# saminiir/level-ip

Hardware: AMD Instinct MI355X
Metric: device-resident checksum GB/s over packet batch; % of HBM-read roofline (higher is better)
Workload: dtype u16

## Files before the change

level-ip_amd/csrc/csum_dev.h:

```cpp
#pragma once

#include <hip/hip_runtime.h>

#include <stdint.h>

#include <atomic>
#include <type_traits>

#include "flat_src.h"
#include "lvlip_csum.h"
#include "lvlip_skb.h"

namespace lvlip {


template <bool ODD>
__device__ __forceinline__ uint32_t dword_words(uint32_t x) {
    if (ODD) x = ((x & 0x00ff00ffu) << 8) | ((x >> 8) & 0x00ff00ffu);
    return (x & 0xffffu) + (x >> 16);
}

template <bool ODD>
__device__ __forceinline__ uint32_t chunk_words(const uint4 v) {
    return dword_words<ODD>(v.x) + dword_words<ODD>(v.y) + dword_words<ODD>(v.z) +
// ... 157 lines not shown
}

template <int G, int WPB = SW_WAVES>
struct Deal {
    uint64_t nw, rank, p_lo;
    uint32_t cnt;

    __device__ __forceinline__ bool init(uint32_t n, uint32_t wid) {
        nw = (uint64_t)gridDim.x * WPB;
        if (G == 0) {
            rank = (uint64_t)blockIdx.x * WPB + wid;
            const uint64_t per = ((uint64_t)n + nw - 1) / nw;
            p_lo = rank * per;
            if (p_lo >= n) return false;
            cnt = (uint32_t)min<uint64_t>(per, (uint64_t)n - p_lo);
            return true;
        }
        rank = (gridDim.x & 7u) == 0u
                   ? ((uint64_t)(blockIdx.x & 7u) * (gridDim.x >> 3) + (blockIdx.x >> 3)) * WPB + wid
                   : (uint64_t)blockIdx.x * WPB + wid;
        p_lo = 0;
        const uint64_t ng = ((uint64_t)n + G - 1) / G;
        if (rank >= ng) return false;
        const uint64_t gcount = (ng - 1 - rank) / nw + 1;
        const uint64_t glast = rank + (gcount - 1) * nw;
        const uint64_t last_size = min<uint64_t>((uint64_t)(G > 0 ? G : 1), (uint64_t)n - glast * G);
        cnt = (uint32_t)((gcount - 1) * G + last_size);
        return true;
    }
    __device__ __forceinline__ uint64_t gidx(uint32_t k) const {
        if (G == 0) return p_lo + k;
        return ((uint64_t)(k / (G > 0 ? G : 1)) * nw + rank) * G + (k % (G > 0 ? G : 1));
    }
};

template <int G, int WPB>
__device__ __forceinline__ void fetch_window(const lvlip_csum_desc* __restrict__ descs,
                                             const Deal<G, WPB>& dl, uint32_t first, uint32_t lane,
                                             uint4* win ) {
    uint32_t k = first + lane;
    k = k < dl.cnt ? k : dl.cnt - 1u;
    const lvlip_csum_desc* g = descs + dl.gidx(k);
    const uint32_t lds = (uint32_t)__builtin_amdgcn_readfirstlane(
        (int)(uint32_t)(uintptr_t)(__attribute__((address_space(3))) uint4*)win);
#pragma clang diagnostic push
#pragma clang diagnostic ignored "-Winline-asm"
    asm volatile("s_nop 4\n\ts_mov_b32 m0, %1\n\ts_nop 0\n\tglobal_load_lds_dwordx4 %0, off"
                 :
                 : "v"(g), "s"(lds)
                 : "memory", "m0");
#pragma clang diagnostic pop
}

template <int R, int G, int POL, int WPB = SW_WAVES>
__device__ __forceinline__ void ring_sweep(const uint8_t* __restrict__ base,
                                           const lvlip_csum_desc* __restrict__ descs, uint32_t n,
                                           uint16_t* __restrict__ out, uint4 (*s_win)[64]) {
    constexpr uint32_t END = 0xffffffffu;
    constexpr uint32_t PIECE = 2048u;
    const uint32_t lane = threadIdx.x & 63u;
    const uint32_t lane16 = lane * 16u;
    const uint32_t wid = uniform(threadIdx.x >> 6);
    Deal<G, WPB> dl;
    if (!dl.init(n, wid)) return;
    const uint32_t cnt = dl.cnt;

    fetch_window<G, WPB>(descs, dl, 0u, lane, s_win[0]);
    fetch_window<G, WPB>(descs, dl, 64u, lane, s_win[1]);
    asm volatile("s_waitcnt vmcnt(0)" ::: "memory");

    uint32_t m_x, m_y, m_z, m_t, m_s;
    auto load_window_meta = [&](uint32_t w) {
        const uint4 d = s_win[w & 1u][lane];
        const PacketMeta pm = packet_meta(base, u32x4{d.x, d.y, d.z, d.w});
        m_x = pm.srd.x;
        m_y = pm.srd.y;
        m_z = pm.srd.z;
        m_t = pm.tinfo;
        m_s = pm.start;
    };
    load_window_meta(0);

    uint32_t ip = 0, io = 0;
    u32x4 srd;
    uint32_t tinfo, start;
    auto pull = [&](uint32_t k) {
        srd.x = (uint32_t)__builtin_amdgcn_readlane((int)m_x, (int)k);
        srd.y = (uint32_t)__builtin_amdgcn_readlane((int)m_y, (int)k);
        srd.z = (uint32_t)__builtin_amdgcn_readlane((int)m_z, (int)k);
        srd.w = SRD_WORD3;
        tinfo = (uint32_t)__builtin_amdgcn_readlane((int)m_t, (int)k);
        start = (uint32_t)__builtin_amdgcn_readlane((int)m_s, (int)k);
    };
    pull(0);

    uint32_t gc = 0;
    uint32_t res_w = 0, res_s = 0;
    uint32_t acc = 0;
    u32x4 va[R], vb[R];
    uint32_t s_pkt[R], s_start[R], s_meta[R];

    auto issue = [&](int r) {
        const bool live = ip < cnt;
        u32x4 sr = srd;
        if (!live) sr.z = 0;
        const uint32_t off = lane16 + io;
        va[r] = buffer_load_nt_asm<POL>(off, sr);
        vb[r] = buffer_load_nt_asm<POL>(off + 1024u, sr);
        const bool last = io + PIECE >= srd.z;
        s_pkt[r] = live ? ip : END;
        s_start[r] = start;
        s_meta[r] = (uint32_t)last | ((tinfo & 3u) << 1) | (((srd.z - 4u) - io) << 3);
        if (live) {
            if (!last) {
                io += PIECE;
            } else {
                ++ip;
                io = 0;
                if (ip < cnt) {
                    if ((ip & 63u) == 0u) {
                        load_window_meta(ip >> 6);
                        fetch_window<G, WPB>(descs, dl, ip + 64u, lane, s_win[((ip >> 6) + 1u) & 1u]);
                    }
                    pull(ip & 63u);
                }
            }
        }
    };

    auto consume = [&](int r) {
        piece_wait<2 * (R - 1)>(va[r], vb[r]);
        u32x4 x = va[r], y = vb[r];
        const uint32_t meta = s_meta[r];
        const uint32_t len3 = (meta >> 1) & 3u;
        if ((meta & 1u) && len3) {
            const uint32_t pos = meta >> 3;
            const uint32_t m = (1u << (8u * len3)) - 1u;
            const bool me = lane == ((pos >> 4) & 63u);
            const uint32_t tk = (pos >> 2) & 3u;
            const bool in_b = pos >= 1024u;
            const uint32_t m0 = (me && tk == 0u) ? m : ~0u, m1 = (me && tk == 1u) ? m : ~0u;
            const uint32_t m2 = (me && tk == 2u) ? m : ~0u, m3 = (me && tk == 3u) ? m : ~0u;
            if (in_b) {
                y.x &= m0; y.y &= m1; y.z &= m2; y.w &= m3;
            } else {
                x.x &= m0; x.y &= m1; x.z &= m2; x.w &= m3;
            }
        }
        acc = dot2_acc(x.x, acc);
        acc = dot2_acc(x.y, acc);
        acc = dot2_acc(x.z, acc);
        acc = dot2_acc(x.w, acc);
        acc = dot2_acc(y.x, acc);
        acc = dot2_acc(y.y, acc);
        acc = dot2_acc(y.z, acc);
        acc = dot2_acc(y.w, acc);
        if (meta & 1u) {
            const uint32_t w = wave_sum_dpp(acc);
            acc = 0;
            const uint32_t k = s_pkt[r] - gc;
            if (lane == k) {
                res_w = w;
                res_s = s_start[r];
            }
            if (k == 63u || s_pkt[r] + 1u == cnt) {
                uint32_t tt = res_s + res_w;
                tt = (tt & 0xffffu) + (tt >> 16);
                tt = (tt & 0xffffu) + (tt >> 16);
                if (lane <= k) out[dl.gidx(gc + lane)] = (uint16_t)~tt;
                gc += 64u;
            }
        }
    };

#pragma unroll
    for (int r = 0; r < R; ++r) issue(r);
    bool done = false;
    while (!done) {
#pragma unroll
        for (int r = 0; r < R; ++r) {
            if (s_pkt[r] == END) {
                done = true;
                break;
            }
            consume(r);
            issue(r);
        }
    }
    asm volatile("s_waitcnt vmcnt(0)" ::: "memory");
}

constexpr int FT = 256;
constexpr uint32_t FCAP = 128;

template <int CTRL>
__device__ __forceinline__ uint32_t dpp_row_shr(uint32_t v) {
    return (uint32_t)__builtin_amdgcn_update_dpp(0, (int)v, CTRL, 0xF, 0xF, false);
}

__device__ __forceinline__ uint32_t wave_incl_scan(uint32_t v) {
    v += dpp_row_shr<0x111>(v);
    v += dpp_row_shr<0x112>(v);
    v += dpp_row_shr<0x114>(v);
    v += dpp_row_shr<0x118>(v);
    v += (uint32_t)__builtin_amdgcn_update_dpp(0, (int)v, 0x142, 0xA, 0xF, false);
    v += (uint32_t)__builtin_amdgcn_update_dpp(0, (int)v, 0x143, 0xC, 0xF, false);
    return v;
}

__device__ __forceinline__ u32x4 group_load_nt(uint64_t a) {
    u32x4 r;
    asm volatile("global_load_dwordx4 %0, %1, off nt" : "=v"(r) : "v"(a) : "memory");
    return r;
}

template <int N>
__device__ __forceinline__ void group_wait(u32x4& a) {
    asm volatile("s_waitcnt vmcnt(%1)" : "+v"(a) : "n"(N) : "memory");
}

__device__ __forceinline__ void block_excl_scan2(uint32_t a, uint32_t b, uint32_t* s_tmp ,
                                                 uint32_t* ea, uint32_t* eb, uint32_t* ta,
                                                 uint32_t* tb) {
    const uint32_t lane = threadIdx.x & 63u, wid = threadIdx.x >> 6;
    const uint32_t ia = wave_incl_scan(a), ib = wave_incl_scan(b);
    if (lane == 63u) {
        s_tmp[wid] = ia;
        s_tmp[4u + wid] = ib;
    }
    __syncthreads();
    uint32_t ba = 0, bb = 0, aa = 0, ab = 0;
#pragma unroll
    for (uint32_t k = 0; k < 4; ++k) {
        const uint32_t x = s_tmp[k], y = s_tmp[4u + k];
        ba += (k < wid) ? x : 0u;
        bb += (k < wid) ? y : 0u;
        aa += x;
        ab += y;
    }
    __syncthreads();
    *ea = ba + ia - a;
    *eb = bb + ib - b;
// ... 557 lines not shown
```

level-ip_amd/csrc/csum_kernels.hip:

```cpp
#include <hip/hip_runtime.h>

#include <stdint.h>
#include <stdio.h>
#include <string.h>

#include "csum_dev.h"

namespace lvlip {

template <int R, int G>
__global__ __launch_bounds__(256) void k_window(const uint8_t* __restrict__ base,
                                                const lvlip_csum_desc* __restrict__ descs,
                                                uint32_t n, uint16_t* __restrict__ out) {
    static_assert(G > 0, "k_window deals groups of G >= 1 packets");
    __shared__ uint4 s_win[SW_WAVES][2][64];
    ring_sweep<R, G, 0>(base, descs, n, out, s_win[uniform(threadIdx.x >> 6)]);
}

template <int S, int P, int K, int M>
__global__ __launch_bounds__(256) void k_lane(const uint8_t* __restrict__ base,
                                              const lvlip_csum_desc* __restrict__ descs,
                                              uint32_t n, uint16_t* __restrict__ out) {
    static_assert(S == 1 || S == 2 || S == 4 || S == 8, "lanes per packet");
    constexpr uint32_t PB = 256 / S;
    const uint32_t lane = threadIdx.x & 63u;
    const uint32_t sub = threadIdx.x & (uint32_t)(S - 1);
    const uint32_t i0 = blockIdx.x * (PB * (uint32_t)P) + threadIdx.x / (uint32_t)S;
    uint4 dd[P];
#pragma unroll
    for (int p = 0; p < P; ++p) {
        const uint32_t i = i0 + PB * p;
        if (M == 0) {
            dd[p] = i < n ? load_global(reinterpret_cast<uint64_t>(descs + i)) : make_uint4(0u, 0u, 0u, 0u);
        } else {
            const uint4 v = load_global(reinterpret_cast<uint64_t>(descs + (i < n ? i : n - 1u)));
            dd[p] = i < n ? v : make_uint4(0u, 0u, 0u, 0u);
        }
    }
    const uint64_t safe = reinterpret_cast<uint64_t>(descs);
    uint64_t a0[P];
    uint32_t lo[P], nch[P], lastv[P];
    uint4 x[P][K];
#pragma unroll
    for (int p = 0; p < P; ++p) {
        const uint64_t abs = reinterpret_cast<uint64_t>(base) + (((uint64_t)dd[p].y << 32) | dd[p].x);
        const int32_t len = (int32_t)dd[p].z;
        a0[p] = abs & ~15ull;
        lo[p] = (uint32_t)(abs & 15ull);
        const uint64_t span = (uint64_t)lo[p] + (uint64_t)(uint32_t)(len > 0 ? len : 0);
        nch[p] = len > 0 ? (uint32_t)((span + 15u) >> 4) : 0u;
        lastv[p] = len > 0 ? (uint32_t)(span - 16ull * (nch[p] - 1u)) : 16u;
        const bool in_group = nch[p] <= (uint32_t)(S * K);
#pragma unroll
        for (int k = 0; k < K; ++k) {
            const uint32_t c = sub + (uint32_t)(S * k);
            const bool want = in_group && c < nch[p];
            if (M == 0)
                x[p][k] = want ? load_nt_global(a0[p] + 16ull * c) : make_uint4(0u, 0u, 0u, 0u);
            else
                x[p][k] = load_nt_global(want ? a0[p] + 16ull * c : safe);
        }
    }
    if (M == 1) __builtin_amdgcn_sched_barrier(0);
    uint32_t acc[P];
#pragma unroll
    for (int p = 0; p < P; ++p) {
        const uint32_t sel = (lo[p] & 1u) ? 0x02030001u : 0x03020100u;
        const bool in_group = nch[p] <= (uint32_t)(S * K);
        uint32_t a = 0;
#pragma unroll
// ... 3 lines not shown
            const int b0 = c == 0u ? (int)lo[p] : 0;
            const int b1 = c + 1u == nch[p] ? (int)lastv[p] : 16;
            if (M == 1 || c == 0u || c + 1u == nch[p]) v = mask_chunk(v, b0, b1);
            a = dot2_acc(__builtin_amdgcn_perm(v.x, v.x, sel), a);
            a = dot2_acc(__builtin_amdgcn_perm(v.y, v.y, sel), a);
            a = dot2_acc(__builtin_amdgcn_perm(v.z, v.z, sel), a);
            a = dot2_acc(__builtin_amdgcn_perm(v.w, v.w, sel), a);
        }
#pragma unroll
        for (int off = 1; off < S; off <<= 1) a += __shfl_xor(a, off, 64);
        acc[p] = a;
    }
#pragma unroll
    for (int p = 0; p < P; ++p) {
        uint64_t big = __builtin_amdgcn_ballot_w64(sub == 0u && nch[p] > (uint32_t)(S * K));
        while (big) {
            const uint32_t q = (uint32_t)__builtin_ctzll(big);
            big &= big - 1ull;
            const uint64_t qa0 = ((uint64_t)(uint32_t)__builtin_amdgcn_readlane((int)(a0[p] >> 32), (int)q) << 32) |
                                 (uint32_t)__builtin_amdgcn_readlane((int)(uint32_t)a0[p], (int)q);
            const uint32_t qlo = (uint32_t)__builtin_amdgcn_readlane((int)lo[p], (int)q);
            const uint32_t qn = (uint32_t)__builtin_amdgcn_readlane((int)nch[p], (int)q);
            const uint32_t qlv = (uint32_t)__builtin_amdgcn_readlane((int)lastv[p], (int)q);
            const uint4* src = reinterpret_cast<const uint4*>(qa0);
            uint32_t w = (qlo & 1u) ? wave_packet_sum<4, true>(src, qn, (int)qlo, qlv, lane)
                                    : wave_packet_sum<4, false>(src, qn, (int)qlo, qlv, lane);
            w = wave_sum_dpp(w);
            if (lane == q) acc[p] = w;
        }
    }
#pragma unroll
    for (int p = 0; p < P; ++p) {
        const uint32_t i = i0 + PB * p;
        if (sub == 0u && i < n) out[i] = finish(dd[p].w, acc[p]);
    }
}

}


namespace {

using lvlip_host::cu_count;
using lvlip_host::current_cus;
using lvlip_host::kLaunchMax;

thread_local char g_last_err[256] = "";

int hip_fail(hipError_t e, const char* what) {
    snprintf(g_last_err, sizeof g_last_err, "%s: %s", what, hipGetErrorString(e));
    return LVLIP_EHIP;
}

template <int R, int G>
void launch_window_g(int waves_per_cu, hipStream_t s, const void* base, const lvlip_csum_desc* d,
                     uint32_t n, uint16_t* out) {
    uint64_t waves = (uint64_t)current_cus() * (uint64_t)waves_per_cu;
    const uint64_t ng = ((uint64_t)n + G - 1) / G;
    if (waves > ng) waves = ng;
    uint64_t grid = (waves + lvlip::SW_WAVES - 1) / lvlip::SW_WAVES;
    if (grid > 8) grid = grid & ~7ull;
    hipLaunchKernelGGL((lvlip::k_window<R, G>), dim3((uint32_t)grid), dim3(256), 0, s,
                       (const uint8_t*)base, d, n, out);
}

int window_group(int requested, int len_hint) {
    if (requested == 1 || requested == 2 || requested == 3 || requested == 4 || requested == 8)
        return requested;
    if (len_hint >= 4096) return 3;
    if (len_hint >= 1792) return 2;
    return 4;
}

template <int R>
void launch_window(int waves_per_cu, hipStream_t s, const void* base, const lvlip_csum_desc* d,
                   uint32_t n, uint16_t* out, int group, int len_hint) {
    switch (window_group(group, len_hint)) {
        case 1: launch_window_g<R, 1>(waves_per_cu, s, base, d, n, out); break;
        case 3: launch_window_g<R, 3>(waves_per_cu, s, base, d, n, out); break;
        case 4: launch_window_g<R, 4>(waves_per_cu, s, base, d, n, out); break;
        case 8: launch_window_g<R, 8>(waves_per_cu, s, base, d, n, out); break;
        default: launch_window_g<R, 2>(waves_per_cu, s, base, d, n, out); break;
    }
}

template <int S, int P, int K>
void launch_lane_spk(int mode, hipStream_t s, const void* base, const lvlip_csum_desc* d, uint32_t n,
                     uint16_t* out) {
    constexpr uint64_t per_block = 256 / S * P;
    const uint32_t grid = (uint32_t)(((uint64_t)n + per_block - 1) / per_block);
    if (mode)
        hipLaunchKernelGGL((lvlip::k_lane<S, P, K, 1>), dim3(grid), dim3(256), 0, s,
                           (const uint8_t*)base, d, n, out);
    else
        hipLaunchKernelGGL((lvlip::k_lane<S, P, K, 0>), dim3(grid), dim3(256), 0, s,
                           (const uint8_t*)base, d, n, out);
}

bool launch_lane(int lanes, int per_group, int chunks, int mode, hipStream_t s, const void* base,
                 const lvlip_csum_desc* d, uint32_t n, uint16_t* out) {
    switch ((lanes << 16) | (chunks << 8) | per_group) {
#define LVLIP_LANE(SS, PP, KK) \
    case (SS << 16) | (KK << 8) | PP: launch_lane_spk<SS, PP, KK>(mode, s, base, d, n, out); return true;
        LVLIP_LANE(1, 2, 4) LVLIP_LANE(1, 4, 4) LVLIP_LANE(1, 2, 6)
        LVLIP_LANE(2, 2, 2) LVLIP_LANE(2, 4, 2) LVLIP_LANE(2, 4, 1) LVLIP_LANE(2, 8, 1)
        LVLIP_LANE(2, 2, 4)
        LVLIP_LANE(4, 2, 1) LVLIP_LANE(4, 4, 1) LVLIP_LANE(4, 8, 1) LVLIP_LANE(4, 2, 2)
        LVLIP_LANE(4, 4, 2)
        LVLIP_LANE(8, 4, 1) LVLIP_LANE(8, 2, 2) LVLIP_LANE(8, 4, 2)
#undef LVLIP_LANE
        default: return false;
    }
}

constexpr int kLaneHintMax = 33;

int auto_select(int hint, uint32_t n, int* unroll, int* wpc) {
    if (hint >= 896) {
        if (*wpc <= 0) *wpc = hint < 1280 ? 16 : (hint < 1792 ? 12 : 8);
        if (*unroll <= 0) {
            const uint64_t nw = (uint64_t)current_cus() * (uint64_t)*wpc;
            int g = hint < 1792 ? 4 : (hint < 4096 ? 2 : 3);
            while (g > 1 && (uint64_t)n < 16ull * (uint64_t)g * nw) --g;
            *unroll = 2 | (g << 8);
        }
        return LVLIP_KERNEL_WINDOW;
    }
    if (hint > 0 && hint < kLaneHintMax) {
        *unroll = 4 | (2 << 8) | (2 << 16);
        return LVLIP_KERNEL_LANE;
    }
    if (*unroll <= 0) *unroll = (hint > 0 && hint < 40) ? 2 : (hint > 0 && hint < 176) ? 4 : 8;
    return LVLIP_KERNEL_FLAT;
}

// ... 242 lines not shown
```

level-ip_amd/csrc/lab_kernels.hip:

```cpp
#include <hip/hip_runtime.h>

#include <stdint.h>
#include <stdlib.h>
#include <string.h>

#include "csum_dev.h"

namespace lvlip {

template <int R, int POL = 0>
__global__ __launch_bounds__(256) void k_stream(const uint8_t* __restrict__ base,
                                                const lvlip_csum_desc* __restrict__ descs,
                                                uint32_t n, uint16_t* __restrict__ out) {
    __shared__ uint4 s_win[SW_WAVES][2][64];
    ring_sweep<R, 0, POL>(base, descs, n, out, s_win[uniform(threadIdx.x >> 6)]);
}

constexpr uint32_t WCAP = 128;

template <int D>
struct WflatLds {
    uint4 rec[SW_WAVES][D];
    uint2 msk[SW_WAVES][D * WCAP / 64];
    uint32_t acc[SW_WAVES][D];
// ... 156 lines not shown
            bigm &= bigm - 1ull;
            const lvlip_csum_desc d = descs[t * D + q];
            const uint64_t abs = reinterpret_cast<uint64_t>(base) + d.offset;
            const int lo = (int)(abs & 15ull);
            const uint64_t span = (uint64_t)lo + (uint64_t)(uint32_t)d.len;
            const uint32_t nchq = (uint32_t)((span + 15u) >> 4);
            const uint32_t lastv = (uint32_t)(span - 16ull * (nchq - 1u));
            const uint4* src = reinterpret_cast<const uint4*>(abs & ~15ull);
            uint32_t w = (abs & 1ull) ? wave_packet_sum<4, true>(src, nchq, lo, lastv, lane)
                                      : wave_packet_sum<4, false>(src, nchq, lo, lastv, lane);
            w = wave_sum_dpp(w);
            if (lane == 0) s_acc[q] = w;
        }
        lds_sync();

        uint32_t acc = s_acc[lane < (uint32_t)D ? lane : 0u];
        if (meta & (3u << 24)) {
            const bool odd = meta & (1u << 17);
            const int lo = (int)((meta >> 8) & 15u), lastv = (int)((meta >> 12) & 31u);
            uint32_t c = 0;
            if (meta & (1u << 24)) {
                uint4 f = s_edge[2u * lane];
                const int fb1 = (nch == 1u) ? lastv : 16;
                f.x &= ~byte_range_mask(lo, fb1, 0);
                f.y &= ~byte_range_mask(lo, fb1, 1);
                f.z &= ~byte_range_mask(lo, fb1, 2);
                f.w &= ~byte_range_mask(lo, fb1, 3);
                c += odd ? chunk_words<true>(f) : chunk_words<false>(f);
            }
            if (meta & (1u << 25)) {
                uint4 l = s_edge[2u * lane + 1u];
                l.x &= ~byte_range_mask(0, lastv, 0);
                l.y &= ~byte_range_mask(0, lastv, 1);
                l.z &= ~byte_range_mask(0, lastv, 2);
                l.w &= ~byte_range_mask(0, lastv, 3);
                c += odd ? chunk_words<true>(l) : chunk_words<false>(l);
            }
            acc -= c;
        }
        res_prev = finish(start_sum, acc);
        i_prev = i;
        st_prev = mine;
        __builtin_amdgcn_wave_barrier();
    }
    if (st_prev) out[i_prev] = res_prev;
}

template <int U, int W, bool FIN, int PFA = 0, int VAR = 0>
__global__ __launch_bounds__(FT) __attribute__((amdgpu_waves_per_eu(W, 8))) void k_flat2_occ(
    const uint8_t* __restrict__ base, const DescSrc src, uint32_t n) {
    flat2_body<U, true, 2, DescSrc, 1, false, FIN, PFA, VAR>(base, src, n);
}

template <int R, int G, int WPB>
__global__ __launch_bounds__(64 * WPB) void k_window_stamp(const uint8_t* __restrict__ base,
                                                           const lvlip_csum_desc* __restrict__ descs, uint32_t n,
                                                           uint16_t* __restrict__ out, uint64_t* __restrict__ stamps) {
    __shared__ uint4 s_win[WPB][2][64];
    const uint64_t t0 = __builtin_amdgcn_s_memrealtime();
    const uint32_t wid = uniform(threadIdx.x >> 6);
    ring_sweep<R, G, 0, WPB>(base, descs, n, out, s_win[wid]);
    const uint64_t t1 = __builtin_amdgcn_s_memrealtime();
    const uint64_t rank = (gridDim.x & 7u) == 0u
                              ? ((uint64_t)(blockIdx.x & 7u) * (gridDim.x >> 3) + (blockIdx.x >> 3)) * WPB + wid
                              : (uint64_t)blockIdx.x * WPB + wid;
    if ((threadIdx.x & 63u) == 0u) {
        stamps[2 * rank] = t0;
        stamps[2 * rank + 1] = t1;
    }
}

__global__ __launch_bounds__(FT) void k_flat2_stamp(const uint8_t* __restrict__ base, const DescSrc src,
                                                    uint32_t n, uint64_t* __restrict__ stamps) {
    const uint64_t t0 = __builtin_amdgcn_s_memrealtime();
    flat2_body<8, true, 2, DescSrc, 1, false, false, kFlatPrefetchTiles>(base, src, n);
    __syncthreads();
    if (threadIdx.x == 0) {
        uint32_t xcc, hwid;
        asm volatile("s_getreg_b32 %0, hwreg(HW_REG_XCC_ID)" : "=s"(xcc));
        asm volatile("s_getreg_b32 %0, hwreg(HW_REG_HW_ID)" : "=s"(hwid));
        const uint64_t t1 = __builtin_amdgcn_s_memrealtime();
        stamps[4u * blockIdx.x] = t0;
        stamps[4u * blockIdx.x + 1u] = t1;
        stamps[4u * blockIdx.x + 2u] = (uint64_t)(xcc & 0xfu) | ((uint64_t)hwid << 8);
        stamps[4u * blockIdx.x + 3u] = 0;
    }
}

}

namespace {

int load_policy() {
    static const int pol = [] {
        const char* e = getenv("LVLIP_LOAD_POLICY");
        if (!e) return 0;
        if (!strcmp(e, "temporal")) return 1;
        if (!strcmp(e, "nt_sc1")) return 2;
        if (!strcmp(e, "nt_sc0sc1")) return 3;
        if (!strcmp(e, "sc1")) return 4;
        return 0;
    }();
    return pol;
}
bool load_nt() { return load_policy() != 1; }

int flat_group_order() {
    static const int c = [] {
        const char* e = getenv("LVLIP_FLAT_GROUPS");
        if (e && strcmp(e, "interleaved") == 0) return 0;
        if (e && strcmp(e, "quarters") == 0) return 1;
        return 2;
    }();
    return c;
// ... 5 lines not shown
        const long x = e ? atol(e) : 0;
        return (size_t)(x < 0 ? 0 : (x > 131072 ? 131072 : x));
    }();
    return v;
}

template <int U>
void launch_stream(int waves_per_cu, hipStream_t s, const void* base, const lvlip_csum_desc* d,
                   uint32_t n, uint16_t* out) {
    uint64_t waves = (uint64_t)lvlip_host::current_cus() * (uint64_t)waves_per_cu;
    if (waves > n) waves = n;
    waves = (waves + 3) & ~3ull;
    const uint32_t grid = (uint32_t)(waves / 4);
    switch (load_policy()) {
#define LVLIP_STREAM_POL(P)                                                              \
    case P:                                                                              \
        hipLaunchKernelGGL((lvlip::k_stream<U, P>), dim3(grid), dim3(256), 0, s,         \
                           (const uint8_t*)base, d, n, out);                             \
        break;
        LVLIP_STREAM_POL(1)
        LVLIP_STREAM_POL(2)
        LVLIP_STREAM_POL(3)
        LVLIP_STREAM_POL(4)
#undef LVLIP_STREAM_POL
        default:
            hipLaunchKernelGGL((lvlip::k_stream<U, 0>), dim3(grid), dim3(256), 0, s,
                               (const uint8_t*)base, d, n, out);
    }
}

template <int U, int D>
void launch_wflat_ud(int waves_per_cu, hipStream_t s, const void* base, const lvlip_csum_desc* d,
                     uint32_t n, uint16_t* out) {
    uint64_t waves = (uint64_t)lvlip_host::current_cus() * (uint64_t)waves_per_cu;
    const uint64_t nt = ((uint64_t)n + D - 1) / D;
    if (waves > nt) waves = nt;
    uint64_t grid = (waves + lvlip::SW_WAVES - 1) / lvlip::SW_WAVES;
    if (grid > 8) grid = grid & ~7ull;
    hipLaunchKernelGGL((lvlip::k_wflat<U, D>), dim3((uint32_t)grid), dim3(256), 0, s,
                       (const uint8_t*)base, d, n, out);
}

template <int U>
bool launch_wflat(int waves_per_cu, hipStream_t s, const void* base, const lvlip_csum_desc* d,
                  uint32_t n, uint16_t* out, int tile) {
    switch (tile) {
        case 16: launch_wflat_ud<U, 16>(waves_per_cu, s, base, d, n, out); return true;
        case 32: launch_wflat_ud<U, 32>(waves_per_cu, s, base, d, n, out); return true;
        case 64: launch_wflat_ud<U, 64>(waves_per_cu, s, base, d, n, out); return true;
        default: return false;
    }
}

}

namespace {

int lab_dispatch(const void* base, const lvlip_csum_desc* descs, uint32_t n, uint16_t* out, hipStream_t s,
                 const lvlip_launch_cfg* cfg) {
    const int kernel = cfg ? cfg->kernel : -1;
    int unroll = cfg ? cfg->unroll : 0;
    const int wpc = cfg ? cfg->waves_per_cu : 0;
    switch (kernel) {
        case 1: {
            if (unroll <= 0) unroll = 2;
            const int w = wpc > 0 ? wpc : 16;
            switch (unroll) {
                case 2: launch_stream<2>(w, s, base, descs, n, out); break;
                case 3: launch_stream<3>(w, s, base, descs, n, out); break;
                case 4: launch_stream<4>(w, s, base, descs, n, out); break;
                default: return LVLIP_EINVAL;
            }
            break;
        }
        case 9: {
            int u = unroll > 0 ? unroll & 0xff : 0;
            int tile = unroll > 0 ? (unroll >> 8) & 0xff : 0;
            if (u == 0) u = 4;
            if (tile == 0) tile = 32;
            const int w = wpc > 0 ? wpc : 8;
            bool ok = false;
            switch (u) {
                case 2: ok = launch_wflat<2>(w, s, base, descs, n, out, tile); break;
                case 4: ok = launch_wflat<4>(w, s, base, descs, n, out, tile); break;
                case 8: ok = launch_wflat<8>(w, s, base, descs, n, out, tile); break;
                default: break;
            }
            if (!ok) return LVLIP_EINVAL;
            break;
        }
        case 3: {
            const uint32_t grid = (uint32_t)(((uint64_t)n + lvlip::FT - 1) / lvlip::FT);
            if (unroll < 0) unroll = 0;
            if ((unroll >> 12) != 0) return LVLIP_EINVAL;
            if ((unroll >> 11) & 1) {
                if ((unroll >> 8) & 7) return LVLIP_EINVAL;
                switch (unroll & 0xff) {
#define LVLIP_FLAT_PIPE(UU)                                                                        \
    case UU:                                                                                       \
        hipLaunchKernelGGL((lvlip::k_flat2<UU, true, 2, lvlip::DescSrc, 1, true>), dim3(grid),     \
                           dim3(lvlip::FT), 0, s, (const uint8_t*)base, lvlip::DescSrc{descs, out}, n); \
        break;
                    LVLIP_FLAT_PIPE(2) LVLIP_FLAT_PIPE(4) LVLIP_FLAT_PIPE(6) LVLIP_FLAT_PIPE(8)
#undef LVLIP_FLAT_PIPE
                    default: return LVLIP_EINVAL;
                }
// ... 27 lines not shown
                           dim3(lvlip::FT), flat_lds_pad(), s, (const uint8_t*)base,         \
                           lvlip::DescSrc{descs, out}, n);                                  \
        break;
                LVLIP_FLAT(2, true, 1) LVLIP_FLAT(2, true, 0) LVLIP_FLAT(2, true, 2)
                LVLIP_FLAT(2, false, 1) LVLIP_FLAT(2, false, 0) LVLIP_FLAT(2, false, 2)
                LVLIP_FLAT(4, true, 1) LVLIP_FLAT(4, true, 0) LVLIP_FLAT(4, true, 2)
                LVLIP_FLAT(4, false, 1) LVLIP_FLAT(4, false, 0) LVLIP_FLAT(4, false, 2)
                LVLIP_FLAT(8, true, 1) LVLIP_FLAT(8, true, 0) LVLIP_FLAT(8, true, 2)
                LVLIP_FLAT(8, false, 1) LVLIP_FLAT(8, false, 0) LVLIP_FLAT(8, false, 2)
                LVLIP_FLAT(6, true, 1) LVLIP_FLAT(6, true, 2) LVLIP_FLAT(12, true, 1) LVLIP_FLAT(12, true, 2)
#undef LVLIP_FLAT
                default: return LVLIP_EINVAL;
            }
            break;
        }
        case 13: {
            if (unroll < 0 || (unroll >> 22) != 0) return LVLIP_EINVAL;
            const uint32_t grid = (uint32_t)(((uint64_t)n + lvlip::FT - 1) / lvlip::FT);
            switch (unroll) {
#define LVLIP_FPF(PP)                                                                            \
    case 8 | (5 << 8) | (PP << 13):                                                              \
        hipLaunchKernelGGL((lvlip::k_flat2_occ<8, 5, false, PP * 640>), dim3(grid), dim3(lvlip::FT), 0, s, \
                           (const uint8_t*)base, lvlip::DescSrc{descs, out}, n);                 \
        break;
                LVLIP_FPF(1) LVLIP_FPF(2) LVLIP_FPF(4) LVLIP_FPF(7)
#undef LVLIP_FPF
#define LVLIP_FPR(QQ)                                                                            \
    case 8 | (5 << 8) | (2 << 13) | (QQ << 16):                                                  \
        hipLaunchKernelGGL((lvlip::k_flat2_occ<8, 5, false, 1280, QQ>), dim3(grid), dim3(lvlip::FT), 0, s, \
                           (const uint8_t*)base, lvlip::DescSrc{descs, out}, n);                 \
        break;
                LVLIP_FPR(1) LVLIP_FPR(2) LVLIP_FPR(3) LVLIP_FPR(4) LVLIP_FPR(5) LVLIP_FPR(6) LVLIP_FPR(7) LVLIP_FPR(8) LVLIP_FPR(10) LVLIP_FPR(32)
#undef LVLIP_FPR
                case 4 | (8 << 8):
                    hipLaunchKernelGGL((lvlip::k_flat2_occ<4, 8, false, 0>), dim3(grid), dim3(lvlip::FT), 0, s,
                                       (const uint8_t*)base, lvlip::DescSrc{descs, out}, n);
                    break;
                case 4 | (7 << 8) | (2 << 13):
                    hipLaunchKernelGGL((lvlip::k_flat2_occ<4, 7, false, 1280>), dim3(grid), dim3(lvlip::FT), 0,
                                       s, (const uint8_t*)base, lvlip::DescSrc{descs, out}, n);
                    break;
#define LVLIP_FOCC(UU, WW, FF)                                                                   \
    case UU | (WW << 8) | (FF << 12):                                                            \
        hipLaunchKernelGGL((lvlip::k_flat2_occ<UU, WW, FF>), dim3(grid), dim3(lvlip::FT), 0, s,  \
                           (const uint8_t*)base, lvlip::DescSrc{descs, out}, n);                 \
        break;
                LVLIP_FOCC(8, 5, 0) LVLIP_FOCC(8, 5, 1) LVLIP_FOCC(8, 6, 0) LVLIP_FOCC(8, 6, 1)
                LVLIP_FOCC(6, 7, 0) LVLIP_FOCC(6, 7, 1)
#undef LVLIP_FOCC
                default: return LVLIP_EINVAL;
            }
            break;
        }
        default: return LVLIP_EINVAL;
    }
    return hipGetLastError() == hipSuccess ? LVLIP_OK : LVLIP_EHIP;
}

}

extern "C" {

__attribute__((visibility("default"))) int lvlip_lab_flat_stamps(const void* base, const lvlip_csum_desc* descs,
                                                                 uint32_t n, uint16_t* out, uint64_t* stamps,
                                                                 uint64_t stamp_bytes, void* stream) {
    if (!base || !descs || !out || !stamps || n == 0 || n > lvlip_host::kLaunchMax) return LVLIP_EINVAL;
    const uint32_t grid = (uint32_t)(((uint64_t)n + lvlip::FT - 1) / lvlip::FT);
    if ((uint64_t)grid * 32u > stamp_bytes) return LVLIP_EINVAL;
    hipLaunchKernelGGL(lvlip::k_flat2_stamp, dim3(grid), dim3(lvlip::FT), 0, (hipStream_t)stream,
                       (const uint8_t*)base, lvlip::DescSrc{descs, out}, n, stamps);
    return hipGetLastError() == hipSuccess ? (int)grid : LVLIP_EHIP;
}

__attribute__((visibility("default"))) int lvlip_lab_window_stamps(const void* base, const lvlip_csum_desc* descs,
                                                                   uint32_t n, uint16_t* out, uint64_t* stamps,
                                                                   uint64_t stamp_bytes, int waves_per_cu, int wpb,
                                                                   void* stream) {
    if (!base || !descs || !out || !stamps || n == 0 || waves_per_cu <= 0) return LVLIP_EINVAL;
    if (wpb != 4 && wpb != 8 && wpb != 12) return LVLIP_EINVAL;
    uint64_t waves = (uint64_t)lvlip_host::current_cus() * (uint64_t)waves_per_cu;
    const uint64_t ng = ((uint64_t)n + 3) / 4;
    if (waves > ng) waves = ng;
    uint64_t grid = (waves + wpb - 1) / wpb;
    if (grid > 8) grid = grid & ~7ull;
    if (grid * wpb * 16ull > stamp_bytes) return LVLIP_EINVAL;
    hipStream_t s = (hipStream_t)stream;
    switch (wpb) {
        case 4:
            hipLaunchKernelGGL((lvlip::k_window_stamp<2, 4, 4>), dim3((uint32_t)grid), dim3(256), 0, s,
                               (const uint8_t*)base, descs, n, out, stamps);
            break;
        case 8:
            hipLaunchKernelGGL((lvlip::k_window_stamp<2, 4, 8>), dim3((uint32_t)grid), dim3(512), 0, s,
                               (const uint8_t*)base, descs, n, out, stamps);
            break;
        default:
            hipLaunchKernelGGL((lvlip::k_window_stamp<2, 4, 12>), dim3((uint32_t)grid), dim3(768), 0, s,
                               (const uint8_t*)base, descs, n, out, stamps);
    }
    return hipGetLastError() == hipSuccess ? (int)(grid * wpb) : LVLIP_EHIP;
}

__attribute__((visibility("default"))) int lvlip_lab_batch_dev_ex(const void* base,
                                                                  const lvlip_csum_desc* descs, uint32_t n,
                                                                  uint16_t* out, void* stream,
                                                                  const lvlip_launch_cfg* cfg) {
    if (n == 0) return LVLIP_OK;
    if (!base || !descs || !out || n > LVLIP_MAX_BATCH || ((uintptr_t)base & 15u) != 0) return LVLIP_EINVAL;
    for (uint32_t lo = 0; lo < n;) {
        const uint32_t m = n - lo < lvlip_host::kLaunchMax ? n - lo : lvlip_host::kLaunchMax;
        const int rc = lab_dispatch(base, descs + lo, m, out + lo, (hipStream_t)stream, cfg);
        if (rc != LVLIP_OK) return rc;
        lo += m;
    }
    return LVLIP_OK;
}

__attribute__((visibility("default"))) int lvlip_lab_frames_dev(int mode, int variant, void* base,
                                                                const lvlip_frame_desc* frames, uint32_t n,
                                                                uint8_t* out8, void* stream) {
    if (n == 0) return LVLIP_OK;
    if (!base || !frames || n > LVLIP_MAX_BATCH / 2u || ((uintptr_t)base & 15u)) return LVLIP_EINVAL;
    if (mode != 0 && mode != 4 && mode != 5 && !out8) return LVLIP_EINVAL;
    hipStream_t s = (hipStream_t)stream;
    if (mode == 4 || mode == 5) {
        if (n > (1u << 30)) return LVLIP_EINVAL;
#define LVLIP_ECHO(P)                                                                                      \
    case P:                                                                                                \
        if (mode == 4) return lvlip::launch_frames_flat<lvlip::FR_ECHO, 8, 2, 0, 0, P>(base, frames, n, out8, s, false); \
        hipLaunchKernelGGL(lvlip::k_echo_reply<P>, dim3((n + 255u) / 256u), dim3(256), 0, s, (uint8_t*)base,  \
                           frames, n, out8);                                                               \
        return hipGetLastError() == hipSuccess ? LVLIP_OK : LVLIP_EHIP;
        if (mode == 5 && variant == 8) {
            hipLaunchKernelGGL((lvlip::k_echo_reply<0, 3>), dim3((n + 255u) / 256u), dim3(256), 0, s,
                               (uint8_t*)base, frames, n, out8);
            return hipGetLastError() == hipSuccess ? LVLIP_OK : LVLIP_EHIP;
        }
        switch (variant) {
            LVLIP_ECHO(0) LVLIP_ECHO(2) LVLIP_ECHO(3) LVLIP_ECHO(4) LVLIP_ECHO(5) LVLIP_ECHO(6) LVLIP_ECHO(7)
            default: return LVLIP_EINVAL;
        }
#undef LVLIP_ECHO
    }
    if (mode == 0 && variant >= 64) {
        switch (variant) {
            case 64: return lvlip::launch_frames_flat<lvlip::FR_TX, 8, 2, 0, 0, 2>(base, frames, n, out8, s, true);
            case 128: return lvlip::launch_frames_flat<lvlip::FR_TX, 8, 2, 0, 0, 3>(base, frames, n, out8, s, true);
            case 192: return lvlip::launch_frames_flat<lvlip::FR_TX, 8, 2, 0, 0, 4>(base, frames, n, out8, s, true);
            case 256: return lvlip::launch_frames_flat<lvlip::FR_TX, 8, 2, 0, 0, 5>(base, frames, n, out8, s, true);
            case 320: return lvlip::launch_frames_flat<lvlip::FR_TX, 8, 2, 0, 0, 6>(base, frames, n, out8, s, true);
            default: return LVLIP_EINVAL;
// ... 40 lines not shown
```

level-ip_amd/lvlip.py:

```python
from __future__ import annotations

import ctypes
import os
from typing import Optional, Sequence

import numpy as np

HERE = os.path.dirname(os.path.abspath(__file__))
LIB_PATH = os.path.join(HERE, "liblvlip_csum.so")
TESTKIT_PATH = os.path.join(HERE, "liblvlip_testkit.so")
LAB_PATH = os.path.join(HERE, "liblvlip_lab.so")

OK, EINVAL, ENODEV, EHIP, ENOMEM, ERANGE = 0, -1, -2, -3, -4, -5
KERNEL_AUTO, KERNEL_FLAT, KERNEL_WINDOW, KERNEL_LANE = 0, 3, 8, 10
KERNEL_WAVE, KERNEL_WFLAT, KERNEL_FLAT_OCC = 1, 9, 13
LAB_KERNELS = (KERNEL_WAVE, KERNEL_WFLAT, KERNEL_FLAT_OCC)
RETIRED_KERNELS = (2, 4, 5, 6, 7, 11, 12, 14, 15)
REG_DMA, REG_ZEROCOPY = 0, 1
KERNEL_NAMES = {"auto": KERNEL_AUTO, "wave": KERNEL_WAVE, "flat": KERNEL_FLAT, "window": KERNEL_WINDOW,
                "wflat": KERNEL_WFLAT, "lane": KERNEL_LANE, "flat_occ": KERNEL_FLAT_OCC}
KERNEL_LABELS = {v: k for k, v in KERNEL_NAMES.items()}

DESC_DTYPE = np.dtype([("offset", "<u8"), ("len", "<i4"), ("start_sum", "<u4")])
assert DESC_DTYPE.itemsize == 16


class LvlipUnavailable(RuntimeError):
    """liblvlip_csum.so is missing or cannot be loaded."""


class LvlipError(RuntimeError):
    def __init__(self, rc: int, what: str):
        self.rc = rc
        detail = ""
        try:
            detail = _lib.lvlip_last_hip_error().decode()
        except Exception:
            pass
        msg = f"{what}: {_lib.lvlip_strerror(rc).decode()} ({rc})"
        if detail:
            msg += f" [{detail}]"
        super().__init__(msg)


class LaunchCfg(ctypes.Structure):
    _fields_ = [("kernel", ctypes.c_int32), ("unroll", ctypes.c_int32),
                ("waves_per_cu", ctypes.c_int32), ("len_hint", ctypes.c_int32)]


class Iov(ctypes.Structure):
    _fields_ = [("ptr", ctypes.c_void_p), ("len", ctypes.c_int32), ("start_sum", ctypes.c_uint32)]


class Frame(ctypes.Structure):
    _fields_ = [("head", ctypes.c_void_p), ("len", ctypes.c_uint32)]


class CtxStats(ctypes.Structure):
    _fields_ = [("gpu_calls", ctypes.c_uint64), ("cpu_calls", ctypes.c_uint64),
                ("pieces", ctypes.c_uint64), ("h2d_bytes", ctypes.c_uint64)]

    def as_dict(self) -> dict:
        return {k: int(getattr(self, k)) for k, _ in self._fields_}


CPU_MAX_DEFAULT = 16384


RX_OK, RX_NOT_IP, RX_SHORT, RX_BAD_VERSION, RX_BAD_IHL, RX_TTL0, RX_BAD_CSUM, RX_BAD_L4, \
    RX_UNKNOWN_PROTO = range(1, 10)
RX_VERIFY_L4 = 0x1
ECHO_FULL = 0x1
PLAN_MALFORMED = 0xFFFFFFFF
# ... 1229 lines not shown
        _check(_lib.lvlip_tx_checksum(self._h, arr, len(frames)), "lvlip_tx_checksum")
        del keep



_testkit = None


def testkit() -> ctypes.CDLL:
    global _testkit
    if _testkit is None:
        tk = _load(TESTKIT_PATH)
        _stamp(tk, TESTKIT_PATH, "lvlip_testkit_build_id", os.path.join(HERE, "TESTKIT_SOURCES"))
        tk.lvlip_testkit_fill.restype = ctypes.c_int
        tk.lvlip_testkit_fill.argtypes = [ctypes.c_void_p, ctypes.c_uint64, ctypes.c_uint64,
                                          ctypes.c_uint64, ctypes.c_void_p]
        tk.lvlip_testkit_paint.restype = ctypes.c_int
        tk.lvlip_testkit_paint.argtypes = [ctypes.c_void_p, ctypes.c_void_p, ctypes.c_void_p,
                                           ctypes.c_uint32, ctypes.c_void_p]
        _testkit = tk
    return _testkit


_lab = None


def lab() -> ctypes.CDLL:
    global _lab
    if _lab is None:
        lb = _load(LAB_PATH)
        _stamp(lb, LAB_PATH, "lvlip_lab_build_id", os.path.join(HERE, "LAB_SOURCES"))
        lb.lvlip_lab_probe.restype = ctypes.c_int
        lb.lvlip_lab_probe.argtypes = [ctypes.c_void_p, ctypes.c_uint64, ctypes.c_void_p,
                                       ctypes.c_int, ctypes.c_int, ctypes.c_int, ctypes.c_int,
                                       ctypes.c_void_p]
        lb.lvlip_lab_atomics.restype = ctypes.c_int
        lb.lvlip_lab_atomics.argtypes = [ctypes.c_void_p, ctypes.c_void_p, ctypes.c_int, ctypes.c_int,
                                         ctypes.c_uint32, ctypes.c_void_p]
        lb.lvlip_lab_probe_tl.restype = ctypes.c_int
        lb.lvlip_lab_probe_tl.argtypes = [ctypes.c_void_p, ctypes.c_uint64, ctypes.c_void_p,
                                          ctypes.c_int, ctypes.c_int, ctypes.c_uint32,
                                          ctypes.c_void_p, ctypes.c_void_p, ctypes.c_int,
                                          ctypes.c_void_p]
        lb.lvlip_lab_probe_chunk.restype = ctypes.c_int
        lb.lvlip_lab_probe_chunk.argtypes = [ctypes.c_void_p, ctypes.c_uint64, ctypes.c_void_p,
                                             ctypes.c_int, ctypes.c_uint32, ctypes.c_uint32,
                                             ctypes.c_int, ctypes.c_void_p]
        lb.lvlip_lab_batch_dev_ex.restype = ctypes.c_int
        lb.lvlip_lab_batch_dev_ex.argtypes = [ctypes.c_void_p, ctypes.c_void_p, ctypes.c_uint32,
                                              ctypes.c_void_p, ctypes.c_void_p, ctypes.POINTER(LaunchCfg)]
        lb.lvlip_lab_frames_dev.restype = ctypes.c_int
        lb.lvlip_lab_frames_dev.argtypes = [ctypes.c_int, ctypes.c_int, ctypes.c_void_p, ctypes.c_void_p,
                                            ctypes.c_uint32, ctypes.c_void_p, ctypes.c_void_p]
        lb.lvlip_lab_probe_pkwin.restype = ctypes.c_int
        lb.lvlip_lab_probe_pkwin.argtypes = [ctypes.c_void_p, ctypes.c_uint64, ctypes.c_void_p,
                                             ctypes.c_int, ctypes.c_int, ctypes.c_void_p]
        _lab = lb
    return _lab
```

Measured before the change: 6907.

## Add LDS progress board pacing waves via s_setprio in window kernel

Adds a per-block shared-memory scoreboard where each wave posts its packet index at every 64-packet window refill. Each wave counts how many peers are ahead of it and raises or lowers its own scheduling priority with s_setprio, so slow waves catch up and the block's tail is evened out. For MTU-sized packets at 12 waves per CU, the production window launcher now uses one 768-thread block per CU with pacing mode 2. The board costs an LDS read and a ballot per window, and the larger block changes occupancy.

Result: faster. 6991, median of 6 (+1.2%).

```diff
diff --git a/level-ip_amd/csrc/csum_dev.h b/level-ip_amd/csrc/csum_dev.h
--- a/level-ip_amd/csrc/csum_dev.h
+++ b/level-ip_amd/csrc/csum_dev.h
@@ -233,18 +233,28 @@
 #pragma clang diagnostic pop
 }
 
-template <int R, int G, int POL, int WPB = SW_WAVES>
+template <int R, int G, int POL, int WPB = SW_WAVES, int PACE = 0>
 __device__ __forceinline__ void ring_sweep(const uint8_t* __restrict__ base,
                                            const lvlip_csum_desc* __restrict__ descs, uint32_t n,
-                                           uint16_t* __restrict__ out, uint4 (*s_win)[64]) {
+                                           uint16_t* __restrict__ out, uint4 (*s_win)[64],
+                                           uint32_t* s_board = nullptr) {
+    static_assert(PACE >= 0 && PACE <= 2 && WPB <= 64, "one board slot per lane at most");
     constexpr uint32_t END = 0xffffffffu;
     constexpr uint32_t PIECE = 2048u;
     const uint32_t lane = threadIdx.x & 63u;
     const uint32_t lane16 = lane * 16u;
     const uint32_t wid = uniform(threadIdx.x >> 6);
     Deal<G, WPB> dl;
-    if (!dl.init(n, wid)) return;
+    if (!dl.init(n, wid)) {
+        if constexpr (PACE != 0) {
+            if (lane == 0u) s_board[wid] = END;
+        }
+        return;
+    }
     const uint32_t cnt = dl.cnt;
+    if constexpr (PACE != 0) {
+        if (lane == 0u) s_board[wid] = 0u;
+    }
 
     fetch_window<G, WPB>(descs, dl, 0u, lane, s_win[0]);
     fetch_window<G, WPB>(descs, dl, 64u, lane, s_win[1]);
@@ -280,6 +290,22 @@
     uint32_t acc = 0;
     u32x4 va[R], vb[R];
     uint32_t s_pkt[R], s_start[R], s_meta[R];
+
+    auto pace = [&]() {
+        if (lane == 0u) s_board[wid] = ip;
+        const uint32_t a = (uint32_t)(uintptr_t)(__attribute__((address_space(3))) uint32_t*)s_board +
+                           4u * (lane < (uint32_t)WPB ? lane : wid);
+        uint32_t slot;
+        asm volatile("ds_read_b32 %0, %1\n\ts_waitcnt lgkmcnt(0)" : "=&v"(slot) : "v"(a) : "memory");
+        const uint32_t p = (uint32_t)__builtin_popcountll(
+            __builtin_amdgcn_ballot_w64(lane < (uint32_t)WPB && lane != wid && slot >= ip));
+        if (2u * p > (uint32_t)WPB)
+            __builtin_amdgcn_s_setprio(PACE == 2 ? 3 : 0);
+        else if (2u * p + 2u < (uint32_t)WPB)
+            __builtin_amdgcn_s_setprio(0);
+        else
+            __builtin_amdgcn_s_setprio(PACE == 2 ? 1 : 0);
+    };
 
     auto issue = [&](int r) {
         const bool live = ip < cnt;
@@ -300,6 +326,7 @@
                 io = 0;
                 if (ip < cnt) {
                     if ((ip & 63u) == 0u) {
+                        if constexpr (PACE != 0) pace();
                         load_window_meta(ip >> 6);
                         fetch_window<G, WPB>(descs, dl, ip + 64u, lane, s_win[((ip >> 6) + 1u) & 1u]);
                     }
@@ -369,6 +396,24 @@
         }
     }
     asm volatile("s_waitcnt vmcnt(0)" ::: "memory");
+    if constexpr (PACE != 0) {
+        if (lane == 0u) s_board[wid] = END;
+    }
+}
+
+template <int R, int G, int WPB = SW_WAVES, int PACE = 0>
+__global__ __launch_bounds__(64 * WPB) void k_window(const uint8_t* __restrict__ base,
+                                                     const lvlip_csum_desc* __restrict__ descs,
+                                                     uint32_t n, uint16_t* __restrict__ out) {
+    static_assert(G > 0, "k_window deals groups of G >= 1 packets");
+    __shared__ uint4 s_win[WPB][2][64];
+    const uint32_t wid = uniform(threadIdx.x >> 6);
+    if constexpr (PACE != 0) {
+        __shared__ uint32_t s_board[WPB];
+        ring_sweep<R, G, 0, WPB, PACE>(base, descs, n, out, s_win[wid], s_board);
+    } else {
+        ring_sweep<R, G, 0, WPB>(base, descs, n, out, s_win[wid]);
+    }
 }
 
 constexpr int FT = 256;
diff --git a/level-ip_amd/csrc/csum_kernels.hip b/level-ip_amd/csrc/csum_kernels.hip
--- a/level-ip_amd/csrc/csum_kernels.hip
+++ b/level-ip_amd/csrc/csum_kernels.hip
@@ -8,14 +8,6 @@
 
 namespace lvlip {
 
-template <int R, int G>
-__global__ __launch_bounds__(256) void k_window(const uint8_t* __restrict__ base,
-                                                const lvlip_csum_desc* __restrict__ descs,
-                                                uint32_t n, uint16_t* __restrict__ out) {
-    static_assert(G > 0, "k_window deals groups of G >= 1 packets");
-    __shared__ uint4 s_win[SW_WAVES][2][64];
-    ring_sweep<R, G, 0>(base, descs, n, out, s_win[uniform(threadIdx.x >> 6)]);
-}
 
 template <int S, int P, int K, int M>
 __global__ __launch_bounds__(256) void k_lane(const uint8_t* __restrict__ base,
@@ -125,11 +117,22 @@
     return LVLIP_EHIP;
 }
 
+constexpr int kPaceWaves = 12;
+
 template <int R, int G>
 void launch_window_g(int waves_per_cu, hipStream_t s, const void* base, const lvlip_csum_desc* d,
-                     uint32_t n, uint16_t* out) {
+                     uint32_t n, uint16_t* out, bool mtu) {
     uint64_t waves = (uint64_t)current_cus() * (uint64_t)waves_per_cu;
     const uint64_t ng = ((uint64_t)n + G - 1) / G;
+    if constexpr (R == 2) {
+        if (mtu && waves_per_cu == kPaceWaves && waves <= ng) {
+            uint64_t grid = (uint64_t)current_cus();
+            if (grid > 8) grid = grid & ~7ull;
+            hipLaunchKernelGGL((lvlip::k_window<2, G, kPaceWaves, 2>), dim3((uint32_t)grid),
+                               dim3(64 * kPaceWaves), 0, s, (const uint8_t*)base, d, n, out);
+            return;
+        }
+    }
     if (waves > ng) waves = ng;
     uint64_t grid = (waves + lvlip::SW_WAVES - 1) / lvlip::SW_WAVES;
     if (grid > 8) grid = grid & ~7ull;
@@ -148,12 +151,13 @@
 template <int R>
 void launch_window(int waves_per_cu, hipStream_t s, const void* base, const lvlip_csum_desc* d,
                    uint32_t n, uint16_t* out, int group, int len_hint) {
+    const bool mtu = len_hint >= 896 && len_hint < 1792;
     switch (window_group(group, len_hint)) {
-        case 1: launch_window_g<R, 1>(waves_per_cu, s, base, d, n, out); break;
-        case 3: launch_window_g<R, 3>(waves_per_cu, s, base, d, n, out); break;
-        case 4: launch_window_g<R, 4>(waves_per_cu, s, base, d, n, out); break;
-        case 8: launch_window_g<R, 8>(waves_per_cu, s, base, d, n, out); break;
-        default: launch_window_g<R, 2>(waves_per_cu, s, base, d, n, out); break;
+        case 1: launch_window_g<R, 1>(waves_per_cu, s, base, d, n, out, mtu); break;
+        case 3: launch_window_g<R, 3>(waves_per_cu, s, base, d, n, out, mtu); break;
+        case 4: launch_window_g<R, 4>(waves_per_cu, s, base, d, n, out, mtu); break;
+        case 8: launch_window_g<R, 8>(waves_per_cu, s, base, d, n, out, mtu); break;
+        default: launch_window_g<R, 2>(waves_per_cu, s, base, d, n, out, mtu); break;
     }
 }
 
diff --git a/level-ip_amd/csrc/lab_kernels.hip b/level-ip_amd/csrc/lab_kernels.hip
--- a/level-ip_amd/csrc/lab_kernels.hip
+++ b/level-ip_amd/csrc/lab_kernels.hip
@@ -232,14 +232,18 @@
     flat2_body<U, true, 2, DescSrc, 1, false, FIN, PFA, VAR>(base, src, n);
 }
 
-template <int R, int G, int WPB>
+template <int R, int G, int WPB, int PACE = 0>
 __global__ __launch_bounds__(64 * WPB) void k_window_stamp(const uint8_t* __restrict__ base,
                                                            const lvlip_csum_desc* __restrict__ descs, uint32_t n,
                                                            uint16_t* __restrict__ out, uint64_t* __restrict__ stamps) {
     __shared__ uint4 s_win[WPB][2][64];
+    __shared__ uint32_t s_board[WPB];
     const uint64_t t0 = __builtin_amdgcn_s_memrealtime();
     const uint32_t wid = uniform(threadIdx.x >> 6);
-    ring_sweep<R, G, 0, WPB>(base, descs, n, out, s_win[wid]);
+    if constexpr (PACE != 0)
+        ring_sweep<R, G, 0, WPB, PACE>(base, descs, n, out, s_win[wid], s_board);
+    else
+        ring_sweep<R, G, 0, WPB>(base, descs, n, out, s_win[wid]);
     const uint64_t t1 = __builtin_amdgcn_s_memrealtime();
     const uint64_t rank = (gridDim.x & 7u) == 0u
                               ? ((uint64_t)(blockIdx.x & 7u) * (gridDim.x >> 3) + (blockIdx.x >> 3)) * WPB + wid
@@ -351,6 +355,48 @@
     }
 }
 
+uint64_t pace_grid(int wpb, int g, uint32_t n, int grid_req) {
+    const uint64_t ng = ((uint64_t)n + g - 1) / g;
+    uint64_t grid = grid_req > 0 ? (uint64_t)grid_req : (uint64_t)lvlip_host::current_cus();
+    if (grid * wpb > ng) grid = (ng + wpb - 1) / wpb;
+    if (grid > 8) grid = grid & ~7ull;
+    return grid;
+}
+
+template <int G, int WPB>
+void launch_pace_gw(int pace, int grid_req, hipStream_t s, const void* base, const lvlip_csum_desc* d,
+                    uint32_t n, uint16_t* out) {
+    const dim3 grid((uint32_t)pace_grid(WPB, G, n, grid_req)), block(64 * WPB);
+    switch (pace) {
+        case 0:
+            hipLaunchKernelGGL((lvlip::k_window<2, G, WPB, 0>), grid, block, 0, s, (const uint8_t*)base, d, n, out);
+            break;
+        case 1:
+            hipLaunchKernelGGL((lvlip::k_window<2, G, WPB, 1>), grid, block, 0, s, (const uint8_t*)base, d, n, out);
+            break;
+        default:
+            hipLaunchKernelGGL((lvlip::k_window<2, G, WPB, 2>), grid, block, 0, s, (const uint8_t*)base, d, n, out);
+    }
+}
+
+template <int G>
+bool launch_pace_g(int wpb, int pace, int grid_req, hipStream_t s, const void* base,
+                   const lvlip_csum_desc* d, uint32_t n, uint16_t* out) {
+    switch (wpb) {
+        case 8: launch_pace_gw<G, 8>(pace, grid_req, s, base, d, n, out); return true;
+        case 12: launch_pace_gw<G, 12>(pace, grid_req, s, base, d, n, out); return true;
+        case 16: launch_pace_gw<G, 16>(pace, grid_req, s, base, d, n, out); return true;
+        default: return false;
+    }
+}
+
+template <int WPB, int PACE>
+void launch_stamp(uint64_t grid, hipStream_t s, const void* base, const lvlip_csum_desc* d, uint32_t n,
+                  uint16_t* out, uint64_t* stamps) {
+    hipLaunchKernelGGL((lvlip::k_window_stamp<2, 4, WPB, PACE>), dim3((uint32_t)grid), dim3(64 * WPB), 0, s,
+                       (const uint8_t*)base, d, n, out, stamps);
+}
+
 }
 
 namespace {
@@ -484,6 +530,25 @@
             }
             break;
         }
+        case 16: {
+            if (unroll < 0) return LVLIP_EINVAL;
+            const int r = unroll & 0xff, pace = (unroll >> 16) & 0xf, grid_req = unroll >> 20;
+            int g = (unroll >> 8) & 0xff;
+            if ((r != 0 && r != 2) || pace > 2) return LVLIP_EINVAL;
+            if (g == 0) g = 4;
+            const int w = wpc > 0 ? wpc : 12;
+            bool ok = false;
+            switch (g) {
+                case 1: ok = launch_pace_g<1>(w, pace, grid_req, s, base, descs, n, out); break;
+                case 2: ok = launch_pace_g<2>(w, pace, grid_req, s, base, descs, n, out); break;
+                case 3: ok = launch_pace_g<3>(w, pace, grid_req, s, base, descs, n, out); break;
+                case 4: ok = launch_pace_g<4>(w, pace, grid_req, s, base, descs, n, out); break;
+                case 8: ok = launch_pace_g<8>(w, pace, grid_req, s, base, descs, n, out); break;
+                default: break;
+            }
+            if (!ok) return LVLIP_EINVAL;
+            break;
+        }
         default: return LVLIP_EINVAL;
     }
     return hipGetLastError() == hipSuccess ? LVLIP_OK : LVLIP_EHIP;
@@ -507,9 +572,10 @@
 __attribute__((visibility("default"))) int lvlip_lab_window_stamps(const void* base, const lvlip_csum_desc* descs,
                                                                    uint32_t n, uint16_t* out, uint64_t* stamps,
                                                                    uint64_t stamp_bytes, int waves_per_cu, int wpb,
-                                                                   void* stream) {
+                                                                   int pace, void* stream) {
     if (!base || !descs || !out || !stamps || n == 0 || waves_per_cu <= 0) return LVLIP_EINVAL;
-    if (wpb != 4 && wpb != 8 && wpb != 12) return LVLIP_EINVAL;
+    if (wpb != 4 && wpb != 8 && wpb != 12 && wpb != 16) return LVLIP_EINVAL;
+    if (pace < 0 || pace > 2 || (pace != 0 && wpb == 4)) return LVLIP_EINVAL;
     uint64_t waves = (uint64_t)lvlip_host::current_cus() * (uint64_t)waves_per_cu;
     const uint64_t ng = ((uint64_t)n + 3) / 4;
     if (waves > ng) waves = ng;
@@ -517,18 +583,15 @@
     if (grid > 8) grid = grid & ~7ull;
     if (grid * wpb * 16ull > stamp_bytes) return LVLIP_EINVAL;
     hipStream_t s = (hipStream_t)stream;
-    switch (wpb) {
-        case 4:
-            hipLaunchKernelGGL((lvlip::k_window_stamp<2, 4, 4>), dim3((uint32_t)grid), dim3(256), 0, s,
-                               (const uint8_t*)base, descs, n, out, stamps);
-            break;
-        case 8:
-            hipLaunchKernelGGL((lvlip::k_window_stamp<2, 4, 8>), dim3((uint32_t)grid), dim3(512), 0, s,
-                               (const uint8_t*)base, descs, n, out, stamps);
-            break;
-        default:
-            hipLaunchKernelGGL((lvlip::k_window_stamp<2, 4, 12>), dim3((uint32_t)grid), dim3(768), 0, s,
-                               (const uint8_t*)base, descs, n, out, stamps);
+    switch (wpb * 4 + pace) {
+#define LVLIP_STAMP(WW, PP) \
+    case WW * 4 + PP: launch_stamp<WW, PP>(grid, s, base, descs, n, out, stamps); break;
+        LVLIP_STAMP(4, 0)
+        LVLIP_STAMP(8, 0) LVLIP_STAMP(8, 1) LVLIP_STAMP(8, 2)
+        LVLIP_STAMP(12, 0) LVLIP_STAMP(12, 1) LVLIP_STAMP(12, 2)
+        LVLIP_STAMP(16, 0) LVLIP_STAMP(16, 1) LVLIP_STAMP(16, 2)
+#undef LVLIP_STAMP
+        default: return LVLIP_EINVAL;
     }
     return hipGetLastError() == hipSuccess ? (int)(grid * wpb) : LVLIP_EHIP;
 }
diff --git a/level-ip_amd/lvlip.py b/level-ip_amd/lvlip.py
--- a/level-ip_amd/lvlip.py
+++ b/level-ip_amd/lvlip.py
@@ -13,12 +13,13 @@
 
 OK, EINVAL, ENODEV, EHIP, ENOMEM, ERANGE = 0, -1, -2, -3, -4, -5
 KERNEL_AUTO, KERNEL_FLAT, KERNEL_WINDOW, KERNEL_LANE = 0, 3, 8, 10
-KERNEL_WAVE, KERNEL_WFLAT, KERNEL_FLAT_OCC = 1, 9, 13
-LAB_KERNELS = (KERNEL_WAVE, KERNEL_WFLAT, KERNEL_FLAT_OCC)
+KERNEL_WAVE, KERNEL_WFLAT, KERNEL_FLAT_OCC, KERNEL_WINDOW_PACE = 1, 9, 13, 16
+LAB_KERNELS = (KERNEL_WAVE, KERNEL_WFLAT, KERNEL_FLAT_OCC, KERNEL_WINDOW_PACE)
 RETIRED_KERNELS = (2, 4, 5, 6, 7, 11, 12, 14, 15)
 REG_DMA, REG_ZEROCOPY = 0, 1
 KERNEL_NAMES = {"auto": KERNEL_AUTO, "wave": KERNEL_WAVE, "flat": KERNEL_FLAT, "window": KERNEL_WINDOW,
-                "wflat": KERNEL_WFLAT, "lane": KERNEL_LANE, "flat_occ": KERNEL_FLAT_OCC}
+                "wflat": KERNEL_WFLAT, "lane": KERNEL_LANE, "flat_occ": KERNEL_FLAT_OCC,
+                "window_pace": KERNEL_WINDOW_PACE}
 KERNEL_LABELS = {v: k for k, v in KERNEL_NAMES.items()}
 
 DESC_DTYPE = np.dtype([("offset", "<u8"), ("len", "<i4"), ("start_sum", "<u4")])
@@ -1354,6 +1355,10 @@
         lb.lvlip_lab_frames_dev.restype = ctypes.c_int
         lb.lvlip_lab_frames_dev.argtypes = [ctypes.c_int, ctypes.c_int, ctypes.c_void_p, ctypes.c_void_p,
                                             ctypes.c_uint32, ctypes.c_void_p, ctypes.c_void_p]
+        lb.lvlip_lab_window_stamps.restype = ctypes.c_int
+        lb.lvlip_lab_window_stamps.argtypes = [ctypes.c_void_p, ctypes.c_void_p, ctypes.c_uint32,
+                                               ctypes.c_void_p, ctypes.c_void_p, ctypes.c_uint64,
+                                               ctypes.c_int, ctypes.c_int, ctypes.c_int, ctypes.c_void_p]
         lb.lvlip_lab_probe_pkwin.restype = ctypes.c_int
         lb.lvlip_lab_probe_pkwin.argtypes = [ctypes.c_void_p, ctypes.c_uint64, ctypes.c_void_p,
                                              ctypes.c_int, ctypes.c_int, ctypes.c_void_p]
```
